# tho-kn/EgoTAP

Measured on AMD Instinct MI355X. Metric: stereo frames/sec (2D->3D lift, B=256, 256x256), higher is better.
Workload: dtype f32; 1 GPU; UnrealEgo 16-joint lifting head (heatmaps [B,90,64,64] -> joints [B,16,3]), forward only, fp32, batch 256 per GPU, inputs resident in HBM; batch_per_gpu=256, global_batch=256, heatmap=64, parallelism=dp1 (batch shards, no collective)

## Files before the change

### egotap_amd/csrc/attention_f32.h

```cpp
#pragma once
#include "common.h"
#include <math.h>

template <int NW>
struct AttnCfg {
    static constexpr int DH = 128, KT = 32, KLD = DH + 4, THREADS = 64 * NW;
    static constexpr int TILE_FLOATS = KT * KLD + KT * DH;
    static constexpr int OUT_FLOATS = NW * 32 * KLD;
    static constexpr int LDS_BYTES = 4 * (TILE_FLOATS > OUT_FLOATS ? TILE_FLOATS : OUT_FLOATS);
};

template <int NW>
__global__ __launch_bounds__(64 * NW, 2) void attention_f32_kernel(const float* __restrict__ QKV,
                                                                 float* __restrict__ CTX, int N, int heads,
                                                                 int qgroups, float scale_log2e, float* __restrict__ LSE, int ksplit,
                                                                 const float* __restrict__ Qsrc, long ldq, int Nq) {
    using Cfg = AttnCfg<NW>;
    constexpr int DH = Cfg::DH, KT = Cfg::KT, KLD = Cfg::KLD, THREADS = Cfg::THREADS;
    extern __shared__ __attribute__((aligned(16))) float smem[];
    float* Ks = smem;
    float* Vs = smem + KT * KLD;

    const int nblk = gridDim.x, bid = blockIdx.x;
    const int q8 = nblk >> 3, r8 = nblk & 7, x8 = bid & 7;
    const int lin = (x8 < r8 ? x8 * (q8 + 1) : r8 * (q8 + 1) + (x8 - r8) * q8) + (bid >> 3);
    const int split = ksplit > 1 ? lin % ksplit : 0;
    const int lq = ksplit > 1 ? lin / ksplit : lin;
    const int bh = lq / qgroups, qg = lq - bh * qgroups;
    const int b = bh / heads, h = bh - b * heads;

    const int tid = threadIdx.x, lane = tid & 63, wid = tid >> 6;
    const int l31 = lane & 31, lh = lane >> 5;
    const int D = heads * DH;
    const long ld = 3L * D;
    const float* base = QKV + (long)b * N * ld + h * DH;
    const int qb = qg * NW + wid;
    const bool valid = qb * 32 < Nq;
    const int q0 = min(qb * 32, Nq - 32);

    float qreg[64];
    {
        const float* qp = Qsrc + ((long)b * Nq + q0 + l31) * ldq + h * DH + 4 * lh;
#pragma unroll
        for (int t = 0; t < 16; ++t) {
            const f32x4 v = *(const f32x4*)(qp + 8 * t);
            qreg[4 * t + 0] = v[0]; qreg[4 * t + 1] = v[1]; qreg[4 * t + 2] = v[2]; qreg[4 * t + 3] = v[3];
        }
    }
    float m_run = -INFINITY, l_run = 0.f;

    constexpr int PER = KT * (DH / 4) / THREADS;
    f32x4 stg[PER];
    auto tile_req = [&](int kt, int vpart) __attribute__((always_inline)) {
        const float* kp = base + (long)min(kt * KT, N - KT) * ld + D + vpart * D;
#pragma unroll
        for (int i = 0; i < PER; ++i) {
            const int idx = tid + i * THREADS, row = idx >> 5, c4 = idx & 31;
            stg[i] = *(const f32x4*)(kp + (size_t)(unsigned)(row * (int)ld + c4 * 4));
        }
    };
    auto tile_put = [&](int vpart) __attribute__((always_inline)) {
#pragma unroll
        for (int i = 0; i < PER; ++i) {
            const int idx = tid + i * THREADS, row = idx >> 5, c4 = idx & 31;
            if (vpart) *(f32x4*)(Vs + row * DH + c4 * 4) = stg[i];
            else *(f32x4*)(Ks + row * KLD + c4 * 4) = stg[i];
        }
    };
    const int tiles_all = (N + KT - 1) / KT;
    const int overlap = tiles_all * KT - N;
    const int kt0 = ksplit > 1 ? (int)((long)split * tiles_all / ksplit) : 0;
    const int ntiles = ksplit > 1 ? (int)((long)(split + 1) * tiles_all / ksplit) : tiles_all;
    {
        f32x4 stg2[PER];
        const float* vp = base + (long)min(kt0 * KT, N - KT) * ld + 2 * D;
        tile_req(kt0, 0);
#pragma unroll
        for (int i = 0; i < PER; ++i) {
            const int idx = tid + i * THREADS, row = idx >> 5, c4 = idx & 31;
            stg2[i] = *(const f32x4*)(vp + (size_t)(unsigned)(row * (int)ld + c4 * 4));
        }
        tile_put(0);
#pragma unroll
        for (int i = 0; i < PER; ++i) {
            const int idx = tid + i * THREADS, row = idx >> 5, c4 = idx & 31;
            *(f32x4*)(Vs + row * DH + c4 * 4) = stg2[i];
        }
    }
    if (kt0 + 1 < ntiles) tile_req(kt0 + 1, 0);
    f32x16 o[4];
#pragma unroll
    for (int dt = 0; dt < 4; ++dt)
#pragma unroll
        for (int r = 0; r < 16; ++r) o[dt][r] = 0.f;
    __syncthreads();
    constexpr float RESC = 8.0f;
    for (int kt = kt0; kt < ntiles; ++kt) {
        f32x16 s;
// ... 115 lines not shown
static int attention_f32_ksplit(int B, int N, int heads, size_t scratch_floats, int num_cu) {
    const long wgs = (long)B * heads * (((N + 31) / 32 + 1) / 2);
    const int ntiles = (N + 31) / 32;
    for (int k = 8; k >= 2; --k)
        if (ntiles % k == 0 && wgs * k <= 9L * num_cu / 2 && (size_t)k * ((size_t)B * N * heads * 128 + (size_t)B * heads * N) <= scratch_floats) return k;
    return 1;
}

static hipError_t attention_f32_launch(const float* QKV, float* CTX, int B, int N, int heads, hipStream_t stream,
                                       float* LSE = nullptr, float* scratch = nullptr, size_t scratch_floats = 0, int num_cu = 256) {
    constexpr int NW = 2;
    using Cfg = AttnCfg<NW>;
    if (B <= 0) return hipSuccess;
    if (N < 32 || N % 4 != 0) return hipErrorInvalidValue;
    auto kern = attention_f32_kernel<NW>;
    const int qgroups = ((N + 31) / 32 + NW - 1) / NW;
    const float scale_log2e = 1.4426950408889634f / sqrtf(128.0f);
    const long wgs = (long)B * heads * qgroups;
    const int ksplit = scratch != nullptr && LSE == nullptr ? attention_f32_ksplit(B, N, heads, scratch_floats, num_cu) : 1;
    if (ksplit > 1) {
        float* part = scratch;
        float* lse_part = scratch + (size_t)ksplit * B * N * heads * 128;
        hipLaunchKernelGGL(kern, dim3((unsigned)(wgs * ksplit)), dim3(Cfg::THREADS), Cfg::LDS_BYTES, stream, QKV, part, N, heads, qgroups, scale_log2e, lse_part, ksplit,
                           QKV, 3L * heads * Cfg::DH, N);
        hipError_t e = hipGetLastError();
        if (e != hipSuccess) return e;
        const long total = (long)B * N * heads * 32;
        hipLaunchKernelGGL(attention_f32_merge_kernel, dim3((unsigned)((total + 255) / 256)), dim3(256), 0, stream, (const float*)part, (const float*)lse_part, CTX, B, N, heads, ksplit);
        return hipGetLastError();
    }
    hipLaunchKernelGGL(kern, dim3(B * heads * qgroups), dim3(Cfg::THREADS), Cfg::LDS_BYTES, stream, QKV, CTX, N, heads,
                       qgroups, scale_log2e, LSE, 1, QKV, 3L * heads * Cfg::DH, N);
    return hipGetLastError();
}

static hipError_t attention_f32_live_launch(const float* Q, long ldq, int Nq, const float* QKV, float* CTX, int B, int N, int heads, hipStream_t stream) {
    constexpr int NW = 2;
    using Cfg = AttnCfg<NW>;
    if (B <= 0) return hipSuccess;
    if (N < 32 || N % 4 != 0 || Nq < 32 || Nq > N || ldq % 4 != 0) return hipErrorInvalidValue;
    const int qgroups = ((Nq + 31) / 32 + NW - 1) / NW;
    const float scale_log2e = 1.4426950408889634f / sqrtf(128.0f);
    hipLaunchKernelGGL(attention_f32_kernel<NW>, dim3(B * heads * qgroups), dim3(Cfg::THREADS), Cfg::LDS_BYTES, stream, QKV, CTX, N, heads,
                       qgroups, scale_log2e, (float*)nullptr, 1, Q, ldq, Nq);
    return hipGetLastError();
}
```

### egotap_amd/csrc/egotap_abi.hip

```cpp
#include <stdarg.h>
#include <stdio.h>
#include <string.h>

#include <cmath>
#include <string>
#include <unordered_map>
#include <vector>

#include "attention_f32.h"
#include "common.h"
#include "lds_opt_in.h"
#include "conv_f32.h"
#include "conv_bf16.h"
#include "gemm_f32.h"
#include "gemm_bf16.h"
#include "gemm_bf16_dma.h"
#include "gemm_f32_dma.h"
#include "attention_bf16.h"
#include "layernorm.h"
#include "metrics.h"
#include "heatmap_synth.h"
#include "pu_chain.h"
#include "gemm_tn_bf16.h"
#include "train_ops.h"
// ... 449 lines not shown
        : h(h_), s(s_), on(h_ && h_->timing) {
        if (!on) return;
        if (h->ev_used + 2 > h->ev.size()) {
            hipEvent_t a, b;
            if (hipEventCreate(&a) != hipSuccess || hipEventCreate(&b) != hipSuccess) { on = false; return; }
            h->ev.push_back(a);
            h->ev.push_back(b);
        }
        (void)hipEventRecord(h->ev[h->ev_used], s);
        h->rec.push_back({role, kernel, flops});
    }
    ~GemmTimer() {
        if (!on) return;
        (void)hipEventRecord(h->ev[h->ev_used + 1], s);
        h->ev_used += 2;
    }
};

template <class AL> struct AlName;
template <> struct AlName<ALoadPlain> { static constexpr const char* v = "ALoadPlain"; };
template <> struct AlName<ALoadPatch> { static constexpr const char* v = "ALoadPatch"; };
template <> struct AlName<ALoadTokens> { static constexpr const char* v = "ALoadTokens"; };
template <> struct AlName<ALoadLive> { static constexpr const char* v = "ALoadLive"; };
template <> struct AlName<ALoadRot> { static constexpr const char* v = "ALoadRot"; };
template <> struct AlName<ALoadStereo> { static constexpr const char* v = "ALoadStereo"; };
template <> struct AlName<ALoadStereoGated> { static constexpr const char* v = "ALoadStereoGated"; };
template <class E> struct EpiName;
template <> struct EpiName<EpiBias> { static constexpr const char* v = "EpiBias"; };
template <> struct EpiName<EpiBiasRes> { static constexpr const char* v = "EpiBiasRes"; };
template <> struct EpiName<EpiBiasResLive> { static constexpr const char* v = "EpiBiasResLive"; };
template <> struct EpiName<EpiBiasGelu> { static constexpr const char* v = "EpiBiasGelu"; };
template <> struct EpiName<EpiBnLrelu> { static constexpr const char* v = "EpiBnLrelu"; };
template <> struct EpiName<EpiPatch> { static constexpr const char* v = "EpiPatch"; };

template <class Cfg, class AL, class Epi>
static hipError_t gemm(Handle* h, const char* role, const AL& al, const SegMat& W, const Epi& epi, float* C, long ldc,
                       int M, int N, int K, hipStream_t s) {
    static const std::string kname = std::string("gemm_f32_kernel<") + std::to_string(Cfg::BM) + "x" +
                                     std::to_string(Cfg::BN) + "x" + std::to_string(Cfg::BK) + "," + AlName<AL>::v + "," +
                                     EpiName<Epi>::v + ">";
    GemmTimer t(h, s, role, kname.c_str(), 2.0 * M * N * K);
    return gemm_f32_launch<Cfg, AL, Epi>(al, W, epi, C, ldc, M, N, K, s);
}

static int device_cu_count() {
    static int n = 0;
    if (n == 0) {
        int dev = 0, v = 0;
        if (hipGetDevice(&dev) == hipSuccess && hipDeviceGetAttribute(&v, hipDeviceAttributeMultiprocessorCount, dev) == hipSuccess && v > 0) n = v;
        else n = 256;
    }
    return n;
}
// ... 352 lines not shown
    const long tiles = (long)((M + 255) / 256) * tn;
    const int mh = (int)((tiles / cus) * cus / tn) * 256;
    if (N % 256 == 0 && K % 32 == 0 && mh > 0 && mh < M) {
        const double t_round = K * 0.2319 + 5.0;
        const double t_big = (double)((tiles + cus - 1) / cus) * t_round;
        const double t_split = (double)(((long)(mh / 256) * tn + cus - 1) / cus) * t_round + 4.0 + gemm_f32_direct_estimate_us<TileA>(M - mh, N, K, cus);
        if (t_split < t_big) {
            hipError_t e = gemm_big(h, role, al, W, epi, C, ldc, mh, N, K, s);
            if (e != hipSuccess) return e;
            return gemm<TileA>(h, role, rebase(al, mh), W, rebase(epi, mh), C + (long)mh * ldc, ldc, M - mh, N, K, s);
        }
    }
    return gemm_big(h, role, al, W, epi, C, ldc, M, N, K, s);
}

static bool lift_prune_last(Handle* h, int B) {
    const int D = h->D, M = B * h->seq, Nq = h->T * h->ppd * h->ppd;
    if (h->precision != EGOTAP_PREC_F32 || h->debug_stop != 0 || h->cfg.vit_layers < 1 || Nq < 32 || Nq >= h->seq || D % 256 != 0) return false;
    const int cus = device_cu_count();
    if (gemm_small_route(h, true, M, 3 * D, D, D, cus, true).kind != GS_BIG || gemm_small_route(h, true, M, D, D, D, cus).kind != GS_BIG ||
        gemm_small_route(h, true, M, 4 * D, D, 4 * D, cus, true).kind != GS_BIG || gemm_small_route(h, true, M, D, 4 * D, D, cus).kind != GS_BIG)
        return false;
    return attention_f32_ksplit(B, h->seq, h->cfg.vit_heads, SPLITK_FLOATS, cus) == 1;
}

struct LiftFrozen {
    size_t patch, qkv[8], o[8], up[8], dn[8], bias3[8], fc1p, fc1r, total;
};
static bool lift_frozen_route(const Handle* h) { return h->precision == EGOTAP_PREC_BF16 && h->D == 1024 && h->seq % 32 == 0; }
static LiftFrozen lift_frozen_plan(const Handle* h, const LiftParams* p, PrepTable* T) {
    LiftFrozen f{};
    const size_t D = h->D, K1 = (size_t)h->ppd * h->ppd * D, K1r = 2 * (size_t)h->cfg.hm_size * h->cfg.hm_size;
    const int NL = h->cfg.vit_layers;
    size_t o = 0;
    int ns = 0;
    unsigned chunk = 0;
    auto seg = [&](const float* src, size_t elems, size_t elem_bytes, size_t at) {
        const size_t dst = at == (size_t)-1 ? o : at;
        if (at == (size_t)-1) o = al256(o + elems * elem_bytes);
        if (T && ns < PrepTable::MAXS) {
            T->s[ns] = PrepSeg{src, (unsigned long long)dst, (unsigned)(elems / 8), chunk};
            chunk += (unsigned)((elems / 8 + PrepTable::CHUNK8 - 1) / PrepTable::CHUNK8);
        }
        ++ns;
        return dst;
    };
// ... 123 lines not shown
            const int sp = gemm_bf16s_ksplit(BT, 2048, K1, cu, SPLITK_FLOATS);
            if (sp > 1) EGO_HIP(gemm_bf16s_splitk_launch(xt, W1, (long)K1, bnf(p.pos_fc[0], Z1), SPK, sp, BT, 2048, K1, cu, s));
            else EGO_HIP(fc1_nt(h, 0, Yb, W1, (long)K1, bnf(p.pos_fc[0], Z1), BT, cu, s));
            EGO_HIP((fc_gemm(h, "pos_fc2", ALoadPlain{Z1, 2048}, segmat1(p.pos_fc[1].w, 512, 2048), bn(p.pos_fc[1]), Z2, 512, BT, 512, 2048, SPK, s)));
            EGO_HIP((fc_gemm(h, "pos_fc3", ALoadPlain{Z2, 512}, segmat1(p.pos_fc[2].w, hid, 512), bn(p.pos_fc[2]), POSZ, hid, BT, hid, 512, SPK, s)));
        }
        {
            const __bf16* hmb = hmb_ready ? hmb_ready : HIDb;
            const long n8 = (long)B * h->C * HW / 8;
            if (!hmb_ready) hipLaunchKernelGGL(f32_to_bf16_kernel, dim3((unsigned)((n8 + 255) / 256)), dim3(256), 0, s, hm, HIDb, n8);
            if (!frozen) prep(p.rot_fc[0].w, Wb, 2048, 2 * HW);
            const __bf16* W1 = frozen ? FW(fz.fc1r) : Wb;
            EGO_HIP(hipGetLastError());
            const XRot xr{hmb, h->C, J, HW};
            const int sp = gemm_bf16s_ksplit(BT, 2048, 2 * HW, cu, SPLITK_FLOATS);
            if (sp > 1) EGO_HIP(gemm_bf16s_splitk_launch(xr, W1, 2L * HW, bnf(p.rot_fc[0], Z1), SPK, sp, BT, 2048, 2 * HW, cu, s));
            else EGO_HIP(fc1_nt(h, 1, hmb, W1, 2L * HW, bnf(p.rot_fc[0], Z1), BT, cu, s));
            EGO_HIP((fc_gemm(h, "rot_fc2", ALoadPlain{Z1, 2048}, segmat1(p.rot_fc[1].w, 512, 2048), bn(p.rot_fc[1]), Z2, 512, BT, 512, 2048, SPK, s)));
            EGO_HIP((fc_gemm(h, "rot_fc3", ALoadPlain{Z2, 512}, segmat1(p.rot_fc[2].w, hid, 512), bn(p.rot_fc[2]), ROTZ, hid, BT, hid, 512, SPK, s)));
        }
    } else {
    const int NL = h->cfg.vit_layers;
    const bool prune = pose_only && lift_prune_last(h, B);
    EGO_HIP(launch_ln(X, Y, NL > 0 ? p.layer[0].ln1_g : p.lnf_g, NL > 0 ? p.layer[0].ln1_b : p.lnf_b, M, 1e-12f, s));
    for (int i = 0; i < NL; ++i) {
        const auto& L = p.layer[i];
        if (prune && i + 1 == NL) {
            const LiveRows lr{h->seq, h->side, h->ppd, h->grid, h->T};
            const int Nq = h->T * h->ppd * h->ppd, Mc = B * Nq;
            float* Xc = QKV;
            SegMat Wkv; Wkv.p[0] = L.k_w; Wkv.p[1] = L.v_w; Wkv.p[2] = L.v_w; Wkv.seg = D; Wkv.ld = D;
            SegVec bkv; bkv.p[0] = L.k_b; bkv.p[1] = L.v_b; bkv.p[2] = L.v_b; bkv.seg = D;
            EGO_HIP((gemm_big(h, "kv", ALoadPlain{Y, D}, Wkv, EpiBias{bkv}, QKV + D, 3L * D, M, 2 * D, D, s)));
            EGO_HIP((gemm_rounds(h, "q_live", ALoadLive{Y, D, lr}, segmat1(L.q_w, D, D), EpiBias{segvec1(L.q_b, D)}, QKV, 3L * D, Mc, D, D, s)));
            EGO_HIP(attention_f32_live_launch(QKV, 3L * D, Nq, QKV, CTX, B, h->seq, h->cfg.vit_heads, s));
            EGO_HIP((gemm_rounds(h, "attn_out_live", ALoadPlain{CTX, D}, segmat1(L.o_w, D, D), EpiBiasResLive{segvec1(L.o_b, D), X, D, lr}, Xc, D, Mc, D, D, s)));
            EGO_HIP(launch_ln(Xc, Y, L.ln2_g, L.ln2_b, Mc, 1e-12f, s));
            EGO_HIP((gemm_rounds(h, "mlp_up_live", ALoadPlain{Y, D}, segmat1(L.up_w, 4 * D, D), EpiBiasGelu{segvec1(L.up_b, 4 * D)}, HID, 4L * D, Mc, 4 * D, D, s)));
            EGO_HIP((gemm_rounds(h, "mlp_down_live", ALoadPlain{HID, 4L * D}, segmat1(L.dn_w, D, 4 * D), EpiBiasRes{segvec1(L.dn_b, D), Xc, D}, Xc, D, Mc, D, 4 * D, s)));
            EGO_HIP(launch_ln(Xc, Y, p.lnf_g, p.lnf_b, Mc, 1e-12f, s));
            break;
        }
        {
            SegMat Wqkv; Wqkv.p[0] = L.q_w; Wqkv.p[1] = L.k_w; Wqkv.p[2] = L.v_w; Wqkv.seg = D; Wqkv.ld = D;
            SegVec bqkv; bqkv.p[0] = L.q_b; bqkv.p[1] = L.k_b; bqkv.p[2] = L.v_b; bqkv.seg = D;
            EGO_HIP((gemm_small(h, "qkv", ALoadPlain{Y, D}, Wqkv, EpiBias{bqkv}, QKV, 3L * D, M, 3 * D, D, SPK, s)));
        }
        if (h->precision == EGOTAP_PREC_BF16X3 && h->seq % 32 == 0) EGO_HIP(attention_bf16_launch<3>(QKV, CTX, B, h->seq, h->cfg.vit_heads, s));
        else if (h->precision == EGOTAP_PREC_BF16 && h->seq % 32 == 0) EGO_HIP(attention_bf16_launch<1>(QKV, CTX, B, h->seq, h->cfg.vit_heads, s));
        else EGO_HIP(attention_f32_launch(QKV, CTX, B, h->seq, h->cfg.vit_heads, s, nullptr, SPK, SPLITK_FLOATS, device_cu_count()));
        EGO_HIP(gemm_res_ln(h, "attn_out", CTX, D, L.o_w, L.o_b, X, M, D, D, L.ln2_g, L.ln2_b, Y, SPK, s));
        EGO_HIP((gemm_small(h, "mlp_up", ALoadPlain{Y, D}, segmat1(L.up_w, 4 * D, D), EpiBiasGelu{segvec1(L.up_b, 4 * D)}, HID, 4L * D, M, 4 * D, D, SPK, s)));
        const bool last = i + 1 == NL;
        EGO_HIP(gemm_res_ln(h, "mlp_down", HID, 4L * D, L.dn_w, L.dn_b, X, M, D, 4 * D, last ? p.lnf_g : p.layer[i + 1].ln1_g, last ? p.lnf_b : p.layer[i + 1].ln1_b, Y,
                            SPK, s));
        if (h->debug_stop == 2 + i) return EGOTAP_OK;
    }
    auto bn = [](const LiftParams::Fc& f) { return EpiBnLrelu{f.b, f.g, f.beta, f.mean, f.var, 1e-5f, 0.2f}; };
    const bool skinny_fc1 = BT < SKINNY_ROWS || (h->precision == EGOTAP_PREC_F32 && (long)((BT + 255) / 256) * (2048 / 256) < 100);
    {
        const int K1 = h->ppd * h->ppd * D;
        auto fc1 = [&](const auto& al) -> hipError_t {
            if (skinny_fc1 && BT <= 64)
                return gemm_f32_splitk_launch<TileS>(al, segmat1(p.pos_fc[0].w, 2048, K1), bn(p.pos_fc[0]), Z1, 2048, SPK, SPLITK_FLOATS, BT, 2048, K1, s, device_cu_count());
            if (skinny_fc1)
                return gemm_f32_splitk_launch<TileA>(al, segmat1(p.pos_fc[0].w, 2048, K1), bn(p.pos_fc[0]), Z1, 2048, SPK, SPLITK_FLOATS, BT, 2048, K1, s);
            return gemm_big(h, "pos_fc1", al, segmat1(p.pos_fc[0].w, 2048, K1), bn(p.pos_fc[0]), Z1, 2048, BT, 2048, K1, s);
        };
        if (prune) EGO_HIP(fc1(ALoadPlain{Y, (long)K1}));
        else EGO_HIP(fc1(ALoadTokens{Y, h->T, D, h->seq, h->side, h->ppd, h->grid}));
        EGO_HIP((fc_gemm(h, "pos_fc2", ALoadPlain{Z1, 2048}, segmat1(p.pos_fc[1].w, 512, 2048), bn(p.pos_fc[1]), Z2, 512, BT, 512, 2048, SPK, s)));
        EGO_HIP((fc_gemm(h, "pos_fc3", ALoadPlain{Z2, 512}, segmat1(p.pos_fc[2].w, hid, 512), bn(p.pos_fc[2]), POSZ, hid, BT, hid, 512, SPK, s)));
// ... 1443 lines not shown
    hipError_t e = gemm_bf16_dma_launch((const __bf16*)x_bf16, (long)K, Bm, EpiBias{segvec1(b, N)}, y, N, M, N, K, device_cu_count(), (hipStream_t)stream);
    if (e == hipErrorInvalidValue) { egotap_set_error("egotap_linear_bf16_dma: N=%d / K=%d not a multiple of the 256 x 256 x 32 tile", N, K); return EGOTAP_ERR_INVALID; }
    EGO_HIP(e);
    return EGOTAP_OK;
}
#endif

#if EGOTAP_IN(0)
extern "C" int egotap_layernorm_f32(const float* x, float* y, const float* gamma, const float* beta, int rows, int dim,
                                    float eps, void* stream) {
    EGO_CHECK(x && y && gamma && beta, "egotap_layernorm_f32: null argument");
    EGO_CHECK(dim == 1024, "egotap_layernorm_f32: dim must be 1024 (ViT hidden size)");
    EGO_HIP(launch_ln(x, y, gamma, beta, rows, eps, (hipStream_t)stream));
    return EGOTAP_OK;
}
#endif

#if EGOTAP_IN(0)
extern "C" int egotap_attention_f32(const float* qkv, float* ctx, int B, int N, int heads, void* stream) {
    EGO_CHECK(qkv && ctx, "egotap_attention_f32: null argument");
    EGO_CHECK(N >= 32 && N % 4 == 0, "egotap_attention_f32: sequence length must be at least 32 and a multiple of 4 (any heatmap side that is a multiple of 16)");
    EGO_CHECK(heads > 0, "egotap_attention_f32: heads must be positive");
    EGO_HIP(attention_f32_launch(qkv, ctx, B, N, heads, (hipStream_t)stream));
    return EGOTAP_OK;
}
#endif

#if EGOTAP_IN(0)
extern "C" int egotap_pose_metrics(const float* pred, const float* gt, int B, int J, float* mpjpe, float* pa_mpjpe, float* aligned,
                                   void* stream) {
    if (B == 0) return EGOTAP_OK;
    EGO_CHECK(pred && gt && mpjpe && pa_mpjpe, "egotap_pose_metrics: null argument");
    EGO_CHECK(B > 0 && J >= 1 && J <= EGOTAP_MAX_JOINTS, "egotap_pose_metrics: bad shape B=%d J=%d", B, J);
    hipLaunchKernelGGL(pose_metrics_kernel, dim3((B + 63) / 64), dim3(64), 0, (hipStream_t)stream, pred, gt, B, J, mpjpe, pa_mpjpe, aligned);
    EGO_HIP(hipGetLastError());
    return EGOTAP_OK;
}
#endif

#if EGOTAP_IN(0)
extern "C" int egotap_pose_metrics_batch_axes(const float* pred, const float* gt, int B, int J, float* mpjpe, float* pa_mpjpe, float* aligned,
                                              void* stream) {
    EGO_CHECK(pred && gt && mpjpe && pa_mpjpe, "egotap_pose_metrics_batch_axes: null argument");
    EGO_CHECK((B == 2 || B == 3) && J >= 1 && J <= EGOTAP_MAX_JOINTS,
              "egotap_pose_metrics_batch_axes: the reference takes this branch for batches of 2 or 3 frames only (B=%d J=%d)", B, J);
    hipLaunchKernelGGL(pose_metrics_batch_axes_kernel, dim3(1), dim3(64), 0, (hipStream_t)stream, pred, gt, B, J, mpjpe, pa_mpjpe, aligned);
// ... 1658 lines not shown
```

### egotap_amd/csrc/gemm_f32.h

```cpp
#pragma once
#include "common.h"
#include <type_traits>

struct ALoadPlain {
    const float* A;
    long lda;
    struct Row { const float* p; };
    __device__ __forceinline__ Row row(int m) const { return Row{A + (long)m * lda}; }
    __device__ __forceinline__ f32x4 load(const Row& r, int k) const { return *(const f32x4*)(r.p + k); }
    static constexpr bool HAS_PTR = true;
    __device__ __forceinline__ const float* ptr(const Row& r, int k) const { return r.p + k; }
    __host__ bool dma_ok() const { return lda % 4 == 0 && lda < (1L << 21) && ((uintptr_t)A & 15) == 0; }
};

struct ALoadPatch {
    const float* hm;
    int C, S, seq, side, ppd, grid, T;
    const float* zeros = nullptr;
    struct Row { const float* p; };
    static constexpr bool HAS_PTR = true;
    __device__ __forceinline__ const float* ptr(const Row& r, int k) const { return r.p ? r.p + (k >> 4) * S + (k & 15) : zeros + k; }
    __host__ bool dma_ok() const { return zeros != nullptr && S % 4 == 0 && ((uintptr_t)hm & 15) == 0 && ((uintptr_t)zeros & 15) == 0; }
    __device__ __forceinline__ Row row(int m) const {
        const int b = m / seq, tok = m - b * seq;
// ... 33 lines not shown
struct LiveRows {
    int seq, side, ppd, grid, T;
    int m0 = 0;
    __host__ __device__ __forceinline__ long phys(int m) const {
        m += m0;
        const int pp = ppd * ppd, L = T * pp;
        const int b = m / L, r = m - b * L, i = r / pp, s = r - i * pp;
        const int pr = (i / grid) * ppd + s / ppd, pc = (i % grid) * ppd + s % ppd;
        return (long)b * seq + pr * side + pc;
    }
};
struct ALoadLive {
    const float* A;
    long lda;
    LiveRows lr;
    struct Row { const float* p; };
    __device__ __forceinline__ Row row(int m) const { return Row{A + lr.phys(m) * lda}; }
    __device__ __forceinline__ f32x4 load(const Row& r, int k) const { return *(const f32x4*)(r.p + k); }
    static constexpr bool HAS_PTR = true;
    __device__ __forceinline__ const float* ptr(const Row& r, int k) const { return r.p + k; }
    __host__ bool dma_ok() const { return lda % 4 == 0 && lda < (1L << 21) && ((uintptr_t)A & 15) == 0; }
};

struct ALoadRot {
    const float* hm;
    int C, J, HW;
    struct Row { const float* p; };
    __device__ __forceinline__ Row row(int m) const {
        const int T = 2 * J;
        const int b = m / T, t = m - b * T;
        const int eye = t / J, j = t - eye * J;
        return Row{hm + (long)(b * C + 2 * J + eye * 2 * J + j) * HW};
    }
    __device__ __forceinline__ f32x4 load(const Row& r, int k) const {
        const int cs = k / HW;
        return *(const f32x4*)(r.p + (long)cs * J * HW + (k - cs * HW));
    }
    static constexpr bool HAS_PTR = true;
    __device__ __forceinline__ const float* ptr(const Row& r, int k) const {
        const int cs = k / HW;
        return r.p + (long)cs * J * HW + (k - cs * HW);
    }
    __host__ bool dma_ok() const { return HW % 4 == 0 && ((uintptr_t)hm & 15) == 0; }
};

struct ALoadStereo {
// ... 204 lines not shown
};

struct EpiScatterPatch : EpiNone {
    float* hm;
    int C, S, seq, side, ppd, grid, T;
    __device__ __forceinline__ float* dst(int m, int n) const {
        const int b = m / seq, tok = m - b * seq;
        const int pr = tok / side, pc = tok - pr * side;
        const int cell = (pr / ppd) * grid + pc / ppd;
        if (cell >= T) return nullptr;
        return hm + ((long)(b * C + cell) * S + (pr % ppd) * 16 + (n >> 4)) * S + (pc % ppd) * 16 + (n & 15);
    }
};
struct EpiScatterRot : EpiNone {
    float* hm;
    int C, J, HW;
    __device__ __forceinline__ float* dst(int m, int n) const {
        const int T = 2 * J;
        const int b = m / T, t = m - b * T;
        const int eye = t / J, j = t - eye * J, cs = n / HW;
        return hm + (long)(b * C + 2 * J + eye * 2 * J + cs * J + j) * HW + (n - cs * HW);
    }
};
template <class E> struct epi_scatters : std::false_type {};
template <> struct epi_scatters<EpiScatterPatch> : std::true_type {};
template <> struct epi_scatters<EpiScatterRot> : std::true_type {};
template <class Epi>
__device__ __forceinline__ void epi_store(const Epi& epi, float* C, long ldc, int m, int n, float v) {
    if constexpr (epi_scatters<Epi>::value) {
        if (float* p = epi.dst(m, n)) *p = v;
    } else {
        C[(long)m * ldc + n] = v;
    }
}
template <class Epi>
__device__ __forceinline__ void epi_store4(const Epi& epi, float* C, long ldc, int m, int n0, const f32x4& v) {
    if constexpr (epi_scatters<Epi>::value) {
        if (float* p = epi.dst(m, n0)) *(f32x4*)p = v;
    } else {
        *(f32x4*)(C + (long)m * ldc + n0) = v;
    }
}

template <int BM_, int BN_, int BK_, int WM_, int WN_, int MINW_>
struct GemmCfg {
    static constexpr int BM = BM_, BN = BN_, BK = BK_, WM = WM_, WN = WN_, MINW = MINW_;
    static constexpr int THREADS = 64 * WM * WN;
    static constexpr int LDK = BK + 4;
    static constexpr int TM = BM / WM / 32, TN = BN / WN / 32;
    static constexpr int A_V4 = BM * BK / 4 / THREADS;
    static constexpr int B_V4 = BN * BK / 4 / THREADS;
    static constexpr int ROWS_PER_PASS = THREADS / (BK / 4);
    static constexpr int LDS_BYTES = 2 * (BM + BN) * LDK * 4;
    static_assert(BM % (32 * WM) == 0 && BN % (32 * WN) == 0, "wave tile must be a multiple of 32x32");
    static_assert(BK % 8 == 0, "BK multiple of 8");
    static_assert((BM * BK / 4) % THREADS == 0 && (BN * BK / 4) % THREADS == 0, "staging must divide evenly");
};

template <class Cfg, class ALoad, class Epi>
__global__ __launch_bounds__(Cfg::THREADS, Cfg::MINW) void gemm_f32_kernel(
// ... 612 lines not shown
```

### egotap_amd/csrc/gemm_f32_dma.h

```cpp
#pragma once
#include <type_traits>
#include "gemm_f32.h"
#include "lds_dma.h"

struct DmaF32Cfg {
    static constexpr int BM = 256, BN = 256, BK = 16, WM = 4, WN = 2, THREADS = 512, NS = 4, TM = 2, TN = 4;
    static constexpr int ROWB = 64;
    static constexpr int STAGE = (BM + BN) * ROWB;
    static constexpr int ELD = 36, EPATCH = 16 * ELD * 4;
    static constexpr int LDS_BYTES = NS * STAGE + (THREADS / 64) * EPATCH;
    static_assert(LDS_BYTES <= 160 * 1024, "LDS budget");
};

template <class ALoad, class Epi>
__global__ __launch_bounds__(DmaF32Cfg::THREADS, 2) void gemm_f32_dma_kernel(ALoad al, SegMat W, Epi epi, float* C,
                                                                          long ldc, int M, int N, int K, int tiles_m, int tiles_n) {
    using Cfg = DmaF32Cfg;
    constexpr int BM = Cfg::BM, BN = Cfg::BN, BK = Cfg::BK, NS = Cfg::NS, TM = Cfg::TM, TN = Cfg::TN, ROWB = Cfg::ROWB, ELD = Cfg::ELD;
    extern __shared__ __attribute__((aligned(16))) char smem_dmaf[];
    const int tid = threadIdx.x, lane = tid & 63, wid = tid >> 6;
    const int wm = wid / Cfg::WN, wn = wid % Cfg::WN;
    const int l31 = lane & 31, lh = lane >> 5;
    float* Es = (float*)(smem_dmaf + NS * Cfg::STAGE + wid * Cfg::EPATCH);

    const int ntiles = tiles_m * tiles_n, nb = gridDim.x, x8 = blockIdx.x & 7, jb = blockIdx.x >> 3;
    const int nbx = (nb >> 3) + (x8 < (nb & 7) ? 1 : 0);
    const int q8 = ntiles >> 3, r8 = ntiles & 7;
    const int lo_t = x8 < r8 ? x8 * (q8 + 1) : r8 * (q8 + 1) + (x8 - r8) * q8;
    const int cnt = q8 + (x8 < r8 ? 1 : 0);
    const int my_n = cnt > jb ? (cnt - jb + nbx - 1) / nbx : 0;
    const int KT = K / BK;
    const int total = my_n * KT;
    if (total == 0) return;
    auto tile_of = [&](int i, int& tm, int& tn) __attribute__((always_inline)) {
        const int lin = lo_t + jb + i * nbx;
        const int per_group = 8 * tiles_n;
        const int g = lin / per_group, first = g * 8;
        const int gsz = min(tiles_m - first, 8);
        const int in = lin - g * per_group;
        tm = first + in % gsz;
        tn = in / gsz;
    };

    const int drow = lane >> 2, dchunk = (lane & 3) ^ (lane >> 4);
    typename ALoad::Row ra0, ra1;
    constexpr bool SBA = std::is_same<ALoad, ALoadPlain>::value;
    unsigned long long abase = 0, wbase = 0;
    unsigned ao0 = 0, ao1 = 0;
    auto uniform64 = [](const void* p) __attribute__((always_inline)) { return lds_dma_base(p); };
    const unsigned wo0 = (unsigned)(((long)(wid * 16 + drow) * W.ld + dchunk * 4) * 4), wo1 = (unsigned)(((long)((wid + 8) * 16 + drow) * W.ld + dchunk * 4) * 4);
    int l_tile = 0, l_kt = 0;
    auto set_rows = [&](int i) __attribute__((always_inline)) {
        int tm, tn;
        tile_of(i, tm, tn);
        if constexpr (SBA) {
            abase = uniform64(al.A + (long)tm * BM * al.lda);
            const long ld = al.lda * 4;
            ao0 = (unsigned)((long)(min(tm * BM + wid * 16 + drow, M - 1) - tm * BM) * ld + dchunk * 16);
            ao1 = (unsigned)((long)(min(tm * BM + (wid + 8) * 16 + drow, M - 1) - tm * BM) * ld + dchunk * 16);
        } else {
        ra0 = al.row(min(tm * BM + wid * 16 + drow, M - 1));
        ra1 = al.row(min(tm * BM + (wid + 8) * 16 + drow, M - 1));
        }
        const int n0 = tn * BN, sidx = n0 / W.seg;
        const float* wp = (sidx == 0 ? W.p[0] : (sidx == 1 ? W.p[1] : W.p[2])) + (long)(n0 - sidx * W.seg) * W.ld;
        wbase = uniform64(wp);
    };
    set_rows(0);
    const unsigned lds0 = (unsigned)(size_t)(__attribute__((address_space(3))) char*)smem_dmaf;
    auto dma1 = [&](const float* g, unsigned lds_addr) __attribute__((always_inline)) {
        asm volatile("s_mov_b32 m0, %1\n\ts_nop 0\n\tglobal_load_lds_dwordx4 %0, off" ::"v"(g), "s"(__builtin_amdgcn_readfirstlane(lds_addr)) : "memory");
    };
    auto dma1s = [&](unsigned voff, unsigned long long sbase, unsigned lds_addr) __attribute__((always_inline)) {
        asm volatile("s_mov_b32 m0, %2\n\ts_nop 0\n\tglobal_load_lds_dwordx4 %0, %1" ::"v"(voff), "s"(sbase), "s"(__builtin_amdgcn_readfirstlane(lds_addr)) : "memory");
    };
    auto dma_part = [&](int st, int part) __attribute__((always_inline)) {
        const unsigned sa = lds0 + st * Cfg::STAGE + wid * 1024;
        const int k0 = l_kt * BK;
// ... 162 lines not shown
```

### egotap_amd/lib.py

```python
from __future__ import annotations

import ctypes as C
import os

from . import build as _build

ERR_NAMES = {1: "EGOTAP_ERR_INVALID", 2: "EGOTAP_ERR_HIP", 3: "EGOTAP_ERR_UNBOUND", 4: "EGOTAP_ERR_WORKSPACE"}
NET_LIFT, NET_HM_POS, NET_HM_ROT = 0, 1, 2
F32, I64, BF16 = 0, 1, 2
PRECISIONS = {"f32": 0, "bf16x3": 1, "bf16": 2}
ABI_VERSION = 2
RGB_FORMS = {0: "none", 1: "heatmaps", 2: "scratch", 3: "handoff"}


class EgotapConfig(C.Structure):
    _fields_ = [(n, C.c_int32) for n in (
        "struct_bytes", "n_joints_hm", "estimate_head", "hm_size", "hidden", "vit_dim", "vit_heads", "vit_layers",
        "patch", "pu_hidden")] + [("hm_blocks", C.c_int32 * 4)]


class EgotapOcam(C.Structure):
    _fields_ = [("pol", C.c_double * 8), ("invpol", C.c_double * 24)] + [(n, C.c_double) for n in ("xc", "yc", "c", "d", "e", "ue_flip")] + [
        ("n_pol", C.c_int32), ("n_invpol", C.c_int32)]

# ... 57 lines not shown
    "egotap_debug_gemm_bk": (C.c_int, [C.c_int]),
    "egotap_debug_conv_addressing": (C.c_int, [C.c_int]),
    "egotap_set_weight_scratch": (C.c_int, [C.c_void_p, C.c_void_p, C.c_size_t]),
    "egotap_set_act_scratch": (C.c_int, [C.c_void_p, C.c_void_p, C.c_size_t]),
    "egotap_lift_frozen_bytes": (C.c_int, [C.c_void_p, C.POINTER(C.c_size_t)]),
    "egotap_lift_freeze": (C.c_int, [C.c_void_p, C.c_void_p, C.c_size_t, C.c_void_p]),
    "egotap_lift_unfreeze": (C.c_int, [C.c_void_p]),
    "egotap_hm_frozen_bytes": (C.c_int, [C.c_void_p, C.c_int, C.c_int, C.POINTER(C.c_size_t)]),
    "egotap_hm_freeze": (C.c_int, [C.c_void_p, C.c_int, C.c_int, C.c_void_p, C.c_size_t, C.c_void_p]),
    "egotap_hm_unfreeze": (C.c_int, [C.c_void_p, C.c_int]),
    "egotap_hm_workspace_bytes": (C.c_int, [C.c_void_p, C.c_int, C.POINTER(C.c_size_t)]),
    "egotap_hm_forward": (C.c_int, [C.c_void_p, C.c_int, C.c_void_p, C.c_void_p, C.c_int, C.c_void_p, C.c_int64, C.c_void_p,
                                    C.c_size_t, C.c_void_p]),
    "egotap_hm_intermediate": (C.c_int, [C.c_void_p, C.c_int, C.c_char_p, C.POINTER(C.c_size_t), C.POINTER(C.c_int64)]),
    "egotap_hm_forward_bnbatch_workspace_bytes": (C.c_int, [C.c_void_p, C.c_int, C.c_int, C.POINTER(C.c_size_t)]),
    "egotap_hm_forward_bnbatch_intermediate": (C.c_int, [C.c_void_p, C.c_int, C.c_int, C.c_char_p, C.POINTER(C.c_size_t), C.POINTER(C.c_int64)]),
    "egotap_hm_forward_bnbatch": (C.c_int, [C.c_void_p, C.c_int, C.c_void_p, C.c_void_p, C.c_int, C.c_void_p, C.c_int64, C.c_int, C.c_void_p,
                                            C.c_size_t, C.c_void_p]),
    "egotap_linear_f32": (C.c_int, [C.c_void_p] * 4 + [C.c_int] * 4 + [C.c_void_p] * 5 + [C.c_int, C.c_void_p]),
    "egotap_gemm_tile_name": (C.c_char_p, [C.c_int]),
    "egotap_linear_bf16_dma": (C.c_int, [C.c_void_p] * 4 + [C.c_int] * 3 + [C.c_void_p]),
    "egotap_layernorm_f32": (C.c_int, [C.c_void_p] * 4 + [C.c_int, C.c_int, C.c_float, C.c_void_p]),
    "egotap_attention_f32": (C.c_int, [C.c_void_p, C.c_void_p, C.c_int, C.c_int, C.c_int, C.c_void_p]),
    "egotap_pose_metrics": (C.c_int, [C.c_void_p, C.c_void_p, C.c_int, C.c_int, C.c_void_p, C.c_void_p, C.c_void_p, C.c_void_p]),
    "egotap_pose_metrics_batch_axes": (C.c_int, [C.c_void_p, C.c_void_p, C.c_int, C.c_int, C.c_void_p, C.c_void_p, C.c_void_p, C.c_void_p]),
    "egotap_attention": (C.c_int, [C.c_void_p, C.c_void_p, C.c_int, C.c_int, C.c_int, C.c_int, C.c_void_p]),
    "egotap_synth_heatmaps": (C.c_int, [C.c_void_p] * 4 + [C.c_int, C.c_int, C.c_int, C.c_void_p, C.c_void_p, C.c_void_p, C.c_void_p]),
    "egotap_timing_enable": (C.c_int, [C.c_void_p, C.c_int]),
    "egotap_timing_read": (C.c_int, [C.c_void_p, C.POINTER(C.c_int), C.POINTER(C.c_double), C.POINTER(C.c_double)]),
    "egotap_timing_detail": (C.c_char_p, [C.c_void_p]),
    "egotap_train_gemm_nt": (C.c_int, [C.c_void_p, C.c_int, C.c_void_p, C.c_int64, C.c_void_p, C.c_void_p, C.c_void_p, C.c_void_p,
                                       C.c_int, C.c_int, C.c_int, C.c_int, C.c_void_p, C.c_void_p, C.c_int, C.c_void_p]),
    "egotap_debug_wgrad_splits": (C.c_int, [C.c_int, C.c_int64, C.c_int64, C.c_size_t, C.c_int, C.c_int, C.c_double, C.c_double, C.POINTER(C.c_int)]),
    "egotap_train_gemm_tn_bias": (C.c_int, [C.c_void_p, C.c_void_p, C.c_int64, C.c_void_p, C.c_void_p, C.c_void_p, C.c_int, C.c_int, C.c_int, C.c_int,
                                           C.c_void_p, C.c_size_t, C.c_void_p]),
    "egotap_train_gemm_tn": (C.c_int, [C.c_void_p, C.c_int, C.c_void_p, C.c_int64, C.c_void_p, C.c_void_p, C.c_void_p, C.c_int, C.c_int,
                                       C.c_int, C.c_int, C.c_int, C.c_void_p, C.c_size_t, C.c_void_p]),
    "egotap_train_colsum": (C.c_int, [C.c_void_p, C.c_int64, C.c_void_p, C.c_int, C.c_int, C.c_int, C.c_void_p, C.c_size_t, C.c_void_p]),
    "egotap_train_transpose": (C.c_int, [C.c_void_p, C.c_void_p, C.c_int, C.c_int, C.c_int64, C.c_void_p]),
    "egotap_train_add_inplace": (C.c_int, [C.c_void_p, C.c_void_p, C.c_int64, C.c_void_p]),
    "egotap_train_patch_fwd": (C.c_int, [C.c_void_p, C.c_void_p, C.c_int] + [C.c_void_p] * 6),
    "egotap_train_patch_split": (C.c_int, [C.c_void_p, C.c_void_p, C.c_void_p, C.c_void_p, C.c_int, C.c_void_p]),
    "egotap_train_tokens_scatter": (C.c_int, [C.c_void_p, C.c_void_p, C.c_void_p, C.c_int, C.c_void_p]),
    "egotap_train_layernorm_fwd": (C.c_int, [C.c_void_p] * 6 + [C.c_int, C.c_float, C.c_void_p]),
    "egotap_train_layernorm_bwd": (C.c_int, [C.c_void_p] * 9 + [C.c_int, C.c_int, C.c_void_p, C.c_size_t, C.c_void_p]),
    "egotap_train_bn_lrelu_fwd": (C.c_int, [C.c_void_p] * 8 + [C.c_int, C.c_int, C.c_float, C.c_float, C.c_void_p, C.c_size_t, C.c_void_p]),
# ... 383 lines not shown
    B = pl.shape[0]
    if tuple(pl.shape) != (B, J1, 2) or tuple(pr.shape) != (B, J1, 2) or tuple(p3.shape) != (B, J1, 3):
        raise ValueError(f"expected [B, {J1}, 2] x 2 and [B, {J1}, 3] for {joint_preset}")
    dev = pl.device
    par = torch.tensor(parents, dtype=torch.int32, device=dev)
    cat = torch.empty((B, 6 * J, res, res), device=dev)
    plen = torch.empty((B, 2, J), device=dev)
    theta = torch.empty((B, J), device=dev)
    check(load().egotap_synth_heatmaps(_ptr(pl), _ptr(pr), _ptr(p3), _ptr(par), B, J, res, _ptr(cat), _ptr(plen), _ptr(theta), _stream()))
    return {"cat": cat, "gt_heatmap_left": cat[:, :J], "gt_heatmap_right": cat[:, J:2 * J],
            "gt_limb_heatmap_left": cat[:, 2 * J:4 * J], "gt_limb_heatmap_right": cat[:, 4 * J:],
            "gt_plength_left": plen[:, 0].repeat(1, 2), "gt_plength_right": plen[:, 1].repeat(1, 2), "gt_limb_theta": theta}


def layernorm(x, gamma, beta, eps: float = 1e-12):
    import torch
    _need_cuda_f32(x, gamma, beta)
    y = torch.empty_like(x)
    rows = x.numel() // x.shape[-1]
    check(load().egotap_layernorm_f32(_ptr(x), _ptr(y), _ptr(gamma), _ptr(beta), rows, x.shape[-1], eps, _stream()))
    return y


def attention(qkv, B: int, N: int, heads: int, precision: str = "f32"):
    import torch
    _need_cuda_f32(qkv)
    ctx = torch.empty((B * N, heads * 128), device=qkv.device, dtype=torch.float32)
    check(load().egotap_attention(_ptr(qkv), _ptr(ctx), B, N, heads, PRECISIONS[precision], _stream()))
    return ctx
```

### include/egotap_debug.h

```cpp
#ifndef EGOTAP_DEBUG_H
#define EGOTAP_DEBUG_H
#include "egotap.h"

#ifdef __cplusplus
extern "C" {
#endif

int egotap_debug_pu_drop_workgroups(egotap_handle h, int n);

int egotap_lift_debug_stop(egotap_handle h, int stage);

int egotap_debug_gemm_bk(int bk);

int egotap_debug_conv_addressing(int mode);

enum { EGOTAP_RGB_FORM_NONE = 0, EGOTAP_RGB_FORM_HEATMAPS = 1, EGOTAP_RGB_FORM_SCRATCH = 2, EGOTAP_RGB_FORM_HANDOFF = 3 };
int egotap_debug_predict_pose_rgb_form(egotap_handle h, int* form);
int egotap_debug_predict_pose_rgb_intermediate(egotap_handle h, int B, int chunk, const char* name, size_t* offset, int64_t* numel);

int egotap_debug_wgrad_splits(int tiles, int64_t slabs, int64_t n_floats, size_t slab_bytes, int num_cu, int lds_bytes, double slab_us, double fixed_us,
                              int* per);

int egotap_timing_enable(egotap_handle h, int enable);
int egotap_timing_read(egotap_handle h, int* launches, double* total_ms, double* total_flops);
const char* egotap_timing_detail(egotap_handle h);

#ifdef __cplusplus
}
#endif
#endif
```

Measured before the change: 2851 stereo frames/s.

## Compute batch-invariant layer-0 QKV rows once and share them in attention

In the first transformer layer, token rows from index n0 onward are treated as identical across the batch. Their QKV projection is computed once for batch 0, and a row-remapping loader and epilogue project only the per-sample head rows. The attention kernel gains a shared_from argument so queries, keys and values past that index are read from batch 0's slice, cutting the layer-0 QKV GEMM work and memory traffic. This relies on those rows really being batch-independent at layer 0, adds an extra small GEMM launch, and adds scattered row addressing in the DMA GEMM path.

```diff
diff --git a/egotap_amd/csrc/attention_f32.h b/egotap_amd/csrc/attention_f32.h
--- a/egotap_amd/csrc/attention_f32.h
+++ b/egotap_amd/csrc/attention_f32.h
@@ -14,7 +14,7 @@
 __global__ __launch_bounds__(64 * NW, 2) void attention_f32_kernel(const float* __restrict__ QKV,
                                                                  float* __restrict__ CTX, int N, int heads,
                                                                  int qgroups, float scale_log2e, float* __restrict__ LSE, int ksplit,
-                                                                 const float* __restrict__ Qsrc, long ldq, int Nq) {
+                                                                 const float* __restrict__ Qsrc, long ldq, int Nq, int shared_from) {
     using Cfg = AttnCfg<NW>;
     constexpr int DH = Cfg::DH, KT = Cfg::KT, KLD = Cfg::KLD, THREADS = Cfg::THREADS;
     extern __shared__ __attribute__((aligned(16))) float smem[];
@@ -34,13 +34,14 @@
     const int D = heads * DH;
     const long ld = 3L * D;
     const float* base = QKV + (long)b * N * ld + h * DH;
+    const float* base0 = QKV + h * DH;
     const int qb = qg * NW + wid;
     const bool valid = qb * 32 < Nq;
     const int q0 = min(qb * 32, Nq - 32);
 
     float qreg[64];
     {
-        const float* qp = Qsrc + ((long)b * Nq + q0 + l31) * ldq + h * DH + 4 * lh;
+        const float* qp = Qsrc + ((long)(q0 >= shared_from ? 0 : b) * Nq + q0 + l31) * ldq + h * DH + 4 * lh;
 #pragma unroll
         for (int t = 0; t < 16; ++t) {
             const f32x4 v = *(const f32x4*)(qp + 8 * t);
@@ -52,7 +53,7 @@
     constexpr int PER = KT * (DH / 4) / THREADS;
     f32x4 stg[PER];
     auto tile_req = [&](int kt, int vpart) __attribute__((always_inline)) {
-        const float* kp = base + (long)min(kt * KT, N - KT) * ld + D + vpart * D;
+        const float* kp = (kt * KT >= shared_from ? base0 : base) + (long)min(kt * KT, N - KT) * ld + D + vpart * D;
 #pragma unroll
         for (int i = 0; i < PER; ++i) {
             const int idx = tid + i * THREADS, row = idx >> 5, c4 = idx & 31;
@@ -73,7 +74,7 @@
     const int ntiles = ksplit > 1 ? (int)((long)(split + 1) * tiles_all / ksplit) : tiles_all;
     {
         f32x4 stg2[PER];
-        const float* vp = base + (long)min(kt0 * KT, N - KT) * ld + 2 * D;
+        const float* vp = (kt0 * KT >= shared_from ? base0 : base) + (long)min(kt0 * KT, N - KT) * ld + 2 * D;
         tile_req(kt0, 0);
 #pragma unroll
         for (int i = 0; i < PER; ++i) {
@@ -235,7 +236,7 @@
         float* part = scratch;
         float* lse_part = scratch + (size_t)ksplit * B * N * heads * 128;
         hipLaunchKernelGGL(kern, dim3((unsigned)(wgs * ksplit)), dim3(Cfg::THREADS), Cfg::LDS_BYTES, stream, QKV, part, N, heads, qgroups, scale_log2e, lse_part, ksplit,
-                           QKV, 3L * heads * Cfg::DH, N);
+                           QKV, 3L * heads * Cfg::DH, N, N);
         hipError_t e = hipGetLastError();
         if (e != hipSuccess) return e;
         const long total = (long)B * N * heads * 32;
@@ -243,7 +244,20 @@
         return hipGetLastError();
     }
     hipLaunchKernelGGL(kern, dim3(B * heads * qgroups), dim3(Cfg::THREADS), Cfg::LDS_BYTES, stream, QKV, CTX, N, heads,
-                       qgroups, scale_log2e, LSE, 1, QKV, 3L * heads * Cfg::DH, N);
+                       qgroups, scale_log2e, LSE, 1, QKV, 3L * heads * Cfg::DH, N, N);
+    return hipGetLastError();
+}
+
+static hipError_t attention_f32_shared_launch(const float* QKV, float* CTX, int B, int N, int heads, int shared_from, hipStream_t stream) {
+    constexpr int NW = 2;
+    using Cfg = AttnCfg<NW>;
+    if (B <= 0) return hipSuccess;
+    if (N < 32 || N % 4 != 0 || shared_from <= 0 || shared_from > N) return hipErrorInvalidValue;
+    if (shared_from < N && (N % 32 != 0 || shared_from % 32 != 0)) return hipErrorInvalidValue;
+    const int qgroups = ((N + 31) / 32 + NW - 1) / NW;
+    const float scale_log2e = 1.4426950408889634f / sqrtf(128.0f);
+    hipLaunchKernelGGL(attention_f32_kernel<NW>, dim3(B * heads * qgroups), dim3(Cfg::THREADS), Cfg::LDS_BYTES, stream, QKV, CTX, N, heads,
+                       qgroups, scale_log2e, (float*)nullptr, 1, QKV, 3L * heads * Cfg::DH, N, shared_from);
     return hipGetLastError();
 }
 
@@ -255,6 +269,6 @@
     const int qgroups = ((Nq + 31) / 32 + NW - 1) / NW;
     const float scale_log2e = 1.4426950408889634f / sqrtf(128.0f);
     hipLaunchKernelGGL(attention_f32_kernel<NW>, dim3(B * heads * qgroups), dim3(Cfg::THREADS), Cfg::LDS_BYTES, stream, QKV, CTX, N, heads,
-                       qgroups, scale_log2e, (float*)nullptr, 1, Q, ldq, Nq);
+                       qgroups, scale_log2e, (float*)nullptr, 1, Q, ldq, Nq, N);
     return hipGetLastError();
 }
diff --git a/egotap_amd/csrc/egotap_abi.hip b/egotap_amd/csrc/egotap_abi.hip
--- a/egotap_amd/csrc/egotap_abi.hip
+++ b/egotap_amd/csrc/egotap_abi.hip
@@ -495,6 +495,7 @@
 template <> struct AlName<ALoadPatch> { static constexpr const char* v = "ALoadPatch"; };
 template <> struct AlName<ALoadTokens> { static constexpr const char* v = "ALoadTokens"; };
 template <> struct AlName<ALoadLive> { static constexpr const char* v = "ALoadLive"; };
+template <> struct AlName<ALoadHead> { static constexpr const char* v = "ALoadHead"; };
 template <> struct AlName<ALoadRot> { static constexpr const char* v = "ALoadRot"; };
 template <> struct AlName<ALoadStereo> { static constexpr const char* v = "ALoadStereo"; };
 template <> struct AlName<ALoadStereoGated> { static constexpr const char* v = "ALoadStereoGated"; };
@@ -502,6 +503,7 @@
 template <> struct EpiName<EpiBias> { static constexpr const char* v = "EpiBias"; };
 template <> struct EpiName<EpiBiasRes> { static constexpr const char* v = "EpiBiasRes"; };
 template <> struct EpiName<EpiBiasResLive> { static constexpr const char* v = "EpiBiasResLive"; };
+template <> struct EpiName<EpiBiasHead> { static constexpr const char* v = "EpiBiasHead"; };
 template <> struct EpiName<EpiBiasGelu> { static constexpr const char* v = "EpiBiasGelu"; };
 template <> struct EpiName<EpiBnLrelu> { static constexpr const char* v = "EpiBnLrelu"; };
 template <> struct EpiName<EpiPatch> { static constexpr const char* v = "EpiPatch"; };
@@ -900,6 +902,18 @@
         gemm_small_route(h, true, M, 4 * D, D, 4 * D, cus, true).kind != GS_BIG || gemm_small_route(h, true, M, D, 4 * D, D, cus).kind != GS_BIG)
         return false;
     return attention_f32_ksplit(B, h->seq, h->cfg.vit_heads, SPLITK_FLOATS, cus) == 1;
+}
+
+static int lift_share_layer0(Handle* h, int B, bool pose_only) {
+    const int D = h->D, seq = h->seq, rows = h->T / h->grid;
+    if (!pose_only || h->precision != EGOTAP_PREC_F32 || h->debug_stop != 0 || h->cfg.vit_layers < 2) return 0;
+    if (h->T >= h->grid * h->grid || h->T % h->grid != 0 || rows < 1) return 0;
+    const int n0 = rows * h->ppd * h->side;
+    if (n0 % 32 != 0 || seq % 32 != 0 || D % DmaF32Cfg::BN != 0 || D % DmaF32Cfg::BK != 0) return 0;
+    if ((long)B * seq >= (1L << 31) || !HeadRows::make(n0, seq).exact((long)B * n0)) return 0;
+    const int cus = device_cu_count();
+    if (gemm_small_route(h, true, B * seq, 3 * D, D, D, cus, true).kind != GS_BIG || gemm_small_route(h, true, B * n0, 3 * D, D, D, cus, true).kind != GS_BIG) return 0;
+    return attention_f32_ksplit(B, seq, h->cfg.vit_heads, SPLITK_FLOATS, cus) == 1 ? n0 : 0;
 }
 
 struct LiftFrozen {
@@ -1069,6 +1083,7 @@
     } else {
     const int NL = h->cfg.vit_layers;
     const bool prune = pose_only && lift_prune_last(h, B);
+    const int share0 = lift_share_layer0(h, B, pose_only);
     EGO_HIP(launch_ln(X, Y, NL > 0 ? p.layer[0].ln1_g : p.lnf_g, NL > 0 ? p.layer[0].ln1_b : p.lnf_b, M, 1e-12f, s));
     for (int i = 0; i < NL; ++i) {
         const auto& L = p.layer[i];
@@ -1091,10 +1106,21 @@
         {
             SegMat Wqkv; Wqkv.p[0] = L.q_w; Wqkv.p[1] = L.k_w; Wqkv.p[2] = L.v_w; Wqkv.seg = D; Wqkv.ld = D;
             SegVec bqkv; bqkv.p[0] = L.q_b; bqkv.p[1] = L.k_b; bqkv.p[2] = L.v_b; bqkv.seg = D;
+            if (i == 0 && share0 > 0) {
+                const HeadRows hr = HeadRows::make(share0, h->seq);
+                const int Ml = B * share0;
+                {
+                    static const std::string kdma = std::string("gemm_f32_dma_kernel<256x256x16,") + AlName<ALoadHead>::v + "," + EpiName<EpiBiasHead>::v + ">";
+                    GemmTimer t(h, s, "qkv", kdma.c_str(), 2.0 * Ml * 3 * D * D);
+                    EGO_HIP(gemm_f32_dma_launch(ALoadHead{Y, D, hr}, Wqkv, EpiBiasHead{{bqkv}, QKV, 3L * D, hr}, QKV, 3L * D, Ml, 3 * D, D, device_cu_count(), s));
+                }
+                EGO_HIP((gemm<TileA>(h, "qkv_shared", ALoadPlain{Y + (long)share0 * D, D}, Wqkv, EpiBias{bqkv}, QKV + (long)share0 * 3 * D, 3L * D, h->seq - share0, 3 * D, D, s)));
+            } else
             EGO_HIP((gemm_small(h, "qkv", ALoadPlain{Y, D}, Wqkv, EpiBias{bqkv}, QKV, 3L * D, M, 3 * D, D, SPK, s)));
         }
         if (h->precision == EGOTAP_PREC_BF16X3 && h->seq % 32 == 0) EGO_HIP(attention_bf16_launch<3>(QKV, CTX, B, h->seq, h->cfg.vit_heads, s));
         else if (h->precision == EGOTAP_PREC_BF16 && h->seq % 32 == 0) EGO_HIP(attention_bf16_launch<1>(QKV, CTX, B, h->seq, h->cfg.vit_heads, s));
+        else if (i == 0 && share0 > 0) EGO_HIP(attention_f32_shared_launch(QKV, CTX, B, h->seq, h->cfg.vit_heads, share0, s));
         else EGO_HIP(attention_f32_launch(QKV, CTX, B, h->seq, h->cfg.vit_heads, s, nullptr, SPK, SPLITK_FLOATS, device_cu_count()));
         EGO_HIP(gemm_res_ln(h, "attn_out", CTX, D, L.o_w, L.o_b, X, M, D, D, L.ln2_g, L.ln2_b, Y, SPK, s));
         EGO_HIP((gemm_small(h, "mlp_up", ALoadPlain{Y, D}, segmat1(L.up_w, 4 * D, D), EpiBiasGelu{segvec1(L.up_b, 4 * D)}, HID, 4L * D, M, 4 * D, D, SPK, s)));
@@ -2584,6 +2610,17 @@
     EGO_CHECK(N >= 32 && N % 4 == 0, "egotap_attention_f32: sequence length must be at least 32 and a multiple of 4 (any heatmap side that is a multiple of 16)");
     EGO_CHECK(heads > 0, "egotap_attention_f32: heads must be positive");
     EGO_HIP(attention_f32_launch(qkv, ctx, B, N, heads, (hipStream_t)stream));
+    return EGOTAP_OK;
+}
+#endif
+
+#if EGOTAP_IN(0)
+extern "C" int egotap_debug_attention_f32_shared(const float* qkv, float* ctx, int B, int N, int heads, int shared_from, void* stream) {
+    EGO_CHECK(qkv && ctx, "egotap_debug_attention_f32_shared: null argument");
+    EGO_CHECK(B >= 0 && N >= 32 && N % 4 == 0 && heads > 0, "egotap_debug_attention_f32_shared: bad shape B=%d N=%d heads=%d", B, N, heads);
+    EGO_CHECK(shared_from > 0 && shared_from <= N && (shared_from == N || (N % 32 == 0 && shared_from % 32 == 0)),
+              "egotap_debug_attention_f32_shared: shared_from=%d must be N, or a multiple of 32 below N with N a multiple of 32", shared_from);
+    EGO_HIP(attention_f32_shared_launch(qkv, ctx, B, N, heads, shared_from, (hipStream_t)stream));
     return EGOTAP_OK;
 }
 #endif
diff --git a/egotap_amd/csrc/gemm_f32.h b/egotap_amd/csrc/gemm_f32.h
--- a/egotap_amd/csrc/gemm_f32.h
+++ b/egotap_amd/csrc/gemm_f32.h
@@ -79,6 +79,28 @@
     __host__ bool dma_ok() const { return lda % 4 == 0 && lda < (1L << 21) && ((uintptr_t)A & 15) == 0; }
 };
 
+struct HeadRows {
+    int n0, seq;
+    unsigned magic;
+    static HeadRows make(int n0, int seq) { return HeadRows{n0, seq, (unsigned)((1ull << 32) / (unsigned)n0 + 1)}; }
+    bool exact(long rows) const { return n0 > 1 && rows > 0 && (unsigned long long)rows * (unsigned)n0 < (1ull << 32); }
+    __host__ __device__ __forceinline__ long phys(int m) const {
+        const int b = (int)(((unsigned long long)(unsigned)m * magic) >> 32);
+        return (long)b * seq + (m - b * n0);
+    }
+};
+struct ALoadHead {
+    const float* A;
+    long lda;
+    HeadRows hr;
+    struct Row { const float* p; };
+    __device__ __forceinline__ Row row(int m) const { return Row{A + hr.phys(m) * lda}; }
+    __device__ __forceinline__ f32x4 load(const Row& r, int k) const { return *(const f32x4*)(r.p + k); }
+    static constexpr bool HAS_PTR = true;
+    __device__ __forceinline__ const float* ptr(const Row& r, int k) const { return r.p + k; }
+    __host__ bool dma_ok() const { return lda % 4 == 0 && (256L / hr.n0 + 2) * hr.seq * lda * 4 < (1L << 31) && ((uintptr_t)A & 15) == 0; }
+};
+
 struct ALoadRot {
     const float* hm;
     int C, J, HW;
@@ -329,12 +351,24 @@
         return hm + (long)(b * C + 2 * J + eye * 2 * J + cs * J + j) * HW + (n - cs * HW);
     }
 };
+struct EpiBiasHead : EpiBias {
+    float* C;
+    long ldc;
+    HeadRows hr;
+    static constexpr bool DST_ALWAYS = true;
+    __device__ __forceinline__ float* dst(int m, int n) const { return C + hr.phys(m) * ldc + n; }
+};
 template <class E> struct epi_scatters : std::false_type {};
 template <> struct epi_scatters<EpiScatterPatch> : std::true_type {};
 template <> struct epi_scatters<EpiScatterRot> : std::true_type {};
+template <> struct epi_scatters<EpiBiasHead> : std::true_type {};
+template <class E, class = void> struct epi_dst_always : std::false_type {};
+template <class E> struct epi_dst_always<E, std::enable_if_t<E::DST_ALWAYS>> : std::true_type {};
 template <class Epi>
 __device__ __forceinline__ void epi_store(const Epi& epi, float* C, long ldc, int m, int n, float v) {
-    if constexpr (epi_scatters<Epi>::value) {
+    if constexpr (epi_dst_always<Epi>::value) {
+        *epi.dst(m, n) = v;
+    } else if constexpr (epi_scatters<Epi>::value) {
         if (float* p = epi.dst(m, n)) *p = v;
     } else {
         C[(long)m * ldc + n] = v;
@@ -342,7 +376,9 @@
 }
 template <class Epi>
 __device__ __forceinline__ void epi_store4(const Epi& epi, float* C, long ldc, int m, int n0, const f32x4& v) {
-    if constexpr (epi_scatters<Epi>::value) {
+    if constexpr (epi_dst_always<Epi>::value) {
+        *(f32x4*)epi.dst(m, n0) = v;
+    } else if constexpr (epi_scatters<Epi>::value) {
         if (float* p = epi.dst(m, n0)) *(f32x4*)p = v;
     } else {
         *(f32x4*)(C + (long)m * ldc + n0) = v;
diff --git a/egotap_amd/csrc/gemm_f32_dma.h b/egotap_amd/csrc/gemm_f32_dma.h
--- a/egotap_amd/csrc/gemm_f32_dma.h
+++ b/egotap_amd/csrc/gemm_f32_dma.h
@@ -44,7 +44,8 @@
 
     const int drow = lane >> 2, dchunk = (lane & 3) ^ (lane >> 4);
     typename ALoad::Row ra0, ra1;
-    constexpr bool SBA = std::is_same<ALoad, ALoadPlain>::value;
+    constexpr bool HEAD = std::is_same<ALoad, ALoadHead>::value;
+    constexpr bool SBA = std::is_same<ALoad, ALoadPlain>::value || HEAD;
     unsigned long long abase = 0, wbase = 0;
     unsigned ao0 = 0, ao1 = 0;
     auto uniform64 = [](const void* p) __attribute__((always_inline)) { return lds_dma_base(p); };
@@ -53,7 +54,12 @@
     auto set_rows = [&](int i) __attribute__((always_inline)) {
         int tm, tn;
         tile_of(i, tm, tn);
-        if constexpr (SBA) {
+        if constexpr (HEAD) {
+            const long p0 = al.hr.phys(tm * BM), ld = al.lda * 4;
+            abase = uniform64(al.A + p0 * al.lda);
+            ao0 = (unsigned)((al.hr.phys(min(tm * BM + wid * 16 + drow, M - 1)) - p0) * ld + dchunk * 16);
+            ao1 = (unsigned)((al.hr.phys(min(tm * BM + (wid + 8) * 16 + drow, M - 1)) - p0) * ld + dchunk * 16);
+        } else if constexpr (SBA) {
             abase = uniform64(al.A + (long)tm * BM * al.lda);
             const long ld = al.lda * 4;
             ao0 = (unsigned)((long)(min(tm * BM + wid * 16 + drow, M - 1) - tm * BM) * ld + dchunk * 16);
diff --git a/egotap_amd/lib.py b/egotap_amd/lib.py
--- a/egotap_amd/lib.py
+++ b/egotap_amd/lib.py
@@ -103,6 +103,7 @@
     "egotap_linear_bf16_dma": (C.c_int, [C.c_void_p] * 4 + [C.c_int] * 3 + [C.c_void_p]),
     "egotap_layernorm_f32": (C.c_int, [C.c_void_p] * 4 + [C.c_int, C.c_int, C.c_float, C.c_void_p]),
     "egotap_attention_f32": (C.c_int, [C.c_void_p, C.c_void_p, C.c_int, C.c_int, C.c_int, C.c_void_p]),
+    "egotap_debug_attention_f32_shared": (C.c_int, [C.c_void_p, C.c_void_p, C.c_int, C.c_int, C.c_int, C.c_int, C.c_void_p]),
     "egotap_pose_metrics": (C.c_int, [C.c_void_p, C.c_void_p, C.c_int, C.c_int, C.c_void_p, C.c_void_p, C.c_void_p, C.c_void_p]),
     "egotap_pose_metrics_batch_axes": (C.c_int, [C.c_void_p, C.c_void_p, C.c_int, C.c_int, C.c_void_p, C.c_void_p, C.c_void_p, C.c_void_p]),
     "egotap_attention": (C.c_int, [C.c_void_p, C.c_void_p, C.c_int, C.c_int, C.c_int, C.c_int, C.c_void_p]),
@@ -532,6 +533,14 @@
     return y
 
 
+def attention_f32_shared(qkv, B: int, N: int, heads: int, shared_from: int):
+    import torch
+    _need_cuda_f32(qkv)
+    ctx = torch.empty((B * N, heads * 128), device=qkv.device, dtype=torch.float32)
+    check(load().egotap_debug_attention_f32_shared(_ptr(qkv), _ptr(ctx), B, N, heads, shared_from, _stream()))
+    return ctx
+
+
 def attention(qkv, B: int, N: int, heads: int, precision: str = "f32"):
     import torch
     _need_cuda_f32(qkv)
diff --git a/include/egotap_debug.h b/include/egotap_debug.h
--- a/include/egotap_debug.h
+++ b/include/egotap_debug.h
@@ -9,6 +9,8 @@
 int egotap_debug_pu_drop_workgroups(egotap_handle h, int n);
 
 int egotap_lift_debug_stop(egotap_handle h, int stage);
+
+int egotap_debug_attention_f32_shared(const float* qkv, float* ctx, int B, int N, int heads, int shared_from, void* stream);
 
 int egotap_debug_gemm_bk(int bk);
 
```

After: 2884 stereo frames/s, median of 6. 1.01x the previous value.
